# ziwang1121/IEEE

Hardware: NVIDIA B200
Metric: queries/sec (distmat+rank+CMC/mAP) (higher is better)
Workload: dtype f16x3 split of f32 (fp32-equivalent products, f32 accumulate); rank: u32/i32; AP: f64

## Files before the change

ieee_b200/csrc/rank.cu:

```cuda
#include "common.cuh"

namespace ieee {

static constexpr uint64_t kPadKey = ~uint64_t(0);

__device__ __forceinline__ void block_bitonic_sort(uint64_t* s, int n) {
  for (int k = 2; k <= n; k <<= 1) {
    for (int j = k >> 1; j > 0; j >>= 1) {
      __syncthreads();
      for (int i = threadIdx.x; i < n; i += blockDim.x) {
        const int p = i ^ j;
        if (p > i) {
          const uint64_t a = s[i], b = s[p];
          const bool up = (i & k) == 0;
          if ((a > b) == up) { s[i] = b; s[p] = a; }
        }
      }
    }
  }
  __syncthreads();
}
__host__ __device__ __forceinline__ int next_pow2(int x) {
  int p = 1;
  while (p < x) p <<= 1;
// ... 265 lines not shown
  int head = (int)(((16 - (addr & 15)) & 15) >> 2);
  if (head > G) head = G;
  const int nvec = (G - head) >> 2;
  const float4* rv = reinterpret_cast<const float4*>(row + head);
  if constexpr (MODE == COUNT_SEARCH_ATOMIC) {
    int g = tid;
    for (; g + 3 * NT < G; g += 4 * NT) {
      const float d0 = row[g], d1 = row[g + NT], d2 = row[g + 2 * NT], d3 = row[g + 3 * NT];
      count_visit_search<NT>(c, d0, (uint32_t)g);
      count_visit_search<NT>(c, d1, (uint32_t)(g + NT));
      count_visit_search<NT>(c, d2, (uint32_t)(g + 2 * NT));
      count_visit_search<NT>(c, d3, (uint32_t)(g + 3 * NT));
    }
    for (; g < G; g += NT) count_visit_search<NT>(c, row[g], (uint32_t)g);
    return;
  } else {
    auto one = [&](float d, uint32_t g) { if (count_visit<MODE, NT>(c, d)) count_fix<MODE, NT>(c, d, g); };
    for (int g = tid; g < head; g += NT) one(row[g], (uint32_t)g);
    int i = tid;
    for (; i + 3 * NT < nvec; i += 4 * NT) {
      const float4 a0 = __ldcs(rv + i), a1 = __ldcs(rv + i + NT), a2 = __ldcs(rv + i + 2 * NT), a3 = __ldcs(rv + i + 3 * NT);
      uint32_t g0 = (uint32_t)(head + 4 * i);
      one(a0.x, g0); one(a0.y, g0 + 1); one(a0.z, g0 + 2); one(a0.w, g0 + 3);
      g0 += 4 * NT;
      one(a1.x, g0); one(a1.y, g0 + 1); one(a1.z, g0 + 2); one(a1.w, g0 + 3);
      g0 += 4 * NT;
      one(a2.x, g0); one(a2.y, g0 + 1); one(a2.z, g0 + 2); one(a2.w, g0 + 3);
      g0 += 4 * NT;
      one(a3.x, g0); one(a3.y, g0 + 1); one(a3.z, g0 + 2); one(a3.w, g0 + 3);
    }
    for (; i < nvec; i += NT) {
      const float4 a = __ldcs(rv + i);
      const uint32_t g0 = (uint32_t)(head + 4 * i);
      one(a.x, g0); one(a.y, g0 + 1); one(a.z, g0 + 2); one(a.w, g0 + 3);
    }
    for (int g = head + 4 * nvec + tid; g < G; g += NT) one(row[g], (uint32_t)g);
  }
}

struct WarpCount {
  const uint64_t* T;
  const uint16_t* cell;
  uint8_t* col;
  const float* row;
  float lo, scale, top;
  uint32_t g_offset;
  int ties;
};

__host__ __device__ __forceinline__ uint16_t warp_cell_word(int first_bin, int n) {
  return (uint16_t)((first_bin << 7) | (n ? (((n - 1) << 1) | 1) : 0));
}

__device__ __forceinline__ uint32_t warp_cell_index(float d, float lo, float scale, float top) {
  return __float2uint_rd(fminf(fmaf(d - lo, scale, 1.0f), top));
}

__device__ __forceinline__ void warp_bump(WarpCount& c, uint32_t row_off, int delta) {
  atomicAdd(reinterpret_cast<int32_t*>(c.col + row_off), delta);
}

__device__ __forceinline__ void warp_fix(WarpCount& c, float d, uint32_t g) {
  const uint32_t ce = c.cell[warp_cell_index(d, c.lo, c.scale, c.top)];
  if (!(ce & 1u)) return;
  const int tent = (int)(ce >> 7), n = (int)((ce >> 1) & 63u) + 1;
  const uint64_t pe = pack_key(d, g + c.g_offset);
  const uint32_t ke = (uint32_t)(pe >> 32);
  int b = tent, same = 0;
  bool is_thr = false;
#pragma unroll 1
  for (int j = tent; j < tent + n; ++j) {
    const uint64_t t = c.T[j];
    b += (t < pe);
    same += ((uint32_t)(t >> 32) == ke);
    is_thr |= (t == pe);
  }
  if (!is_thr) c.ties += same;
  if (b != tent) {
    warp_bump(c, (uint32_t)tent << 7, -1);
    warp_bump(c, (uint32_t)b << 7, 1);
  }
}

__device__ __forceinline__ void warp_visit8(WarpCount& c, const float4& u, const float4& v, uint32_t& mask) {
  const float d[8] = {u.x, u.y, u.z, u.w, v.x, v.y, v.z, v.w};
  uint32_t ce[8];
#pragma unroll
  for (int e = 0; e < 8; ++e) ce[e] = c.cell[warp_cell_index(d[e], c.lo, c.scale, c.top)];
#pragma unroll
  for (int e = 0; e < 8; ++e) {
    warp_bump(c, ce[e] & 0xFF80u, 1);
    mask = mask * 2u + (ce[e] & 1u);
  }
}

__device__ __forceinline__ void warp_count_stream(WarpCount& c, int G, int lane, int wq, int team) {
  const float* __restrict__ row = c.row;
  const uintptr_t addr = reinterpret_cast<uintptr_t>(row);
  int head = (int)(((16 - (addr & 15)) & 15) >> 2);
  if (head > G) head = G;
  const int nvec = (G - head) >> 2;
  const float4* rv = reinterpret_cast<const float4*>(row + head);
  const int S = 32 * team, t0 = wq * 32 + lane;
  auto one = [&](int g) {
    const float d = row[g];
    const uint32_t ce = c.cell[warp_cell_index(d, c.lo, c.scale, c.top)];
    warp_bump(c, ce & 0xFF80u, 1);
    if (ce & 1u) warp_fix(c, d, (uint32_t)g);
  };
  for (int g = t0; g < head; g += S) one(g);
  int i = t0;
  bool have = i + 3 * S < nvec;
  float4 a0, a1, a2, a3;
  if (have) { a0 = __ldg(rv + i); a1 = __ldg(rv + i + S); a2 = __ldg(rv + i + 2 * S); a3 = __ldg(rv + i + 3 * S); }
  while (have) {
    const int in = i + 4 * S;
    const bool more = in + 3 * S < nvec;
    float4 n0 = a0, n1 = a1, n2 = a2, n3 = a3;
    if (more) { n0 = __ldg(rv + in); n1 = __ldg(rv + in + S); n2 = __ldg(rv + in + 2 * S); n3 = __ldg(rv + in + 3 * S); }
    uint32_t mask = 0;
    warp_visit8(c, a0, a1, mask);
    warp_visit8(c, a2, a3, mask);
#pragma unroll 1
    while (mask) {
      const int bit = 31 - __clz(mask);
      mask &= ~(1u << bit);
      const int e = 15 - bit;
      const int g = head + 4 * (i + (e >> 2) * S) + (e & 3);
      warp_fix(c, __ldg(row + g), (uint32_t)g);
    }
    a0 = n0; a1 = n1; a2 = n2; a3 = n3;
    i = in;
    have = more;
  }
  for (; i < nvec; i += S) {
    const int g0 = head + 4 * i;
    one(g0); one(g0 + 1); one(g0 + 2); one(g0 + 3);
  }
  for (int g = head + 4 * nvec + t0; g < G; g += S) one(g);
}

struct CountRow {
  int32_t* local;
  const PeerView* pv;
  int64_t slot_row;
  __device__ __forceinline__ void put(int idx, int32_t v) const {
    if (pv->shards == 0) { local[idx] = v; return; }
    for (int p = 0; p < pv->shards; ++p) reinterpret_cast<int32_t*>(pv->base[p] + pv->off_cnt)[slot_row + idx] = v;
  }
};
__device__ __forceinline__ CountRow count_row(int32_t* counts, int64_t q, int stride, const PeerView& pv) {
  CountRow r;
  r.local = counts ? counts + q * stride : nullptr;
  r.pv = &pv;
  r.slot_row = ((int64_t)pv.my * pv.Qb + q) * stride;
  return r;
}

constexpr int kWarpQ = 8;
constexpr int kCountTeamDefault = 1;
constexpr int kWarpRmax = 128;
struct WarpMisc { float lo, scale, top; int R, use_lut, ties; uint32_t kmax; int pad; };
__host__ __device__ inline int warp_smem_per_query(int rmax, int wpq) {
  return ((rmax * 8 + (rmax + 2) * 4 + (kLutCells + 4) * 2 + 32 + wpq * (rmax + 2) * 32 * 4) + 15) & ~15;
}

template <int WPQ>
__global__ void __launch_bounds__(32 * kWarpQ)
rank_count_warp_kernel(const float* __restrict__ distmat, int64_t ld, int64_t Q, int G, int64_t g_offset, int shards, int cap,
                       int out_cap, int rmax, const uint64_t* __restrict__ rel_all, const int32_t* __restrict__ n_rel,
                       const uint64_t* __restrict__ junk, const int32_t* __restrict__ n_junk, int32_t* __restrict__ counts,
                       unsigned long long* __restrict__ ties_out, const PeerView pv) {
  static_assert(WPQ == 1 || WPQ == 2 || WPQ == 4 || WPQ == kWarpQ, "1, 2, 4 or all 8 warps of the CTA per query");
  if (pv.shards) peer_signal_and_wait(pv, 0);
  constexpr bool kTeam = WPQ > 1;
  constexpr int kTeams = kWarpQ / WPQ;
  extern __shared__ __align__(16) uint8_t ws_raw[];
  const int lane = threadIdx.x & 31, w = threadIdx.x >> 5;
  const int team = w / WPQ, wq = w % WPQ;
  uint8_t* mine = ws_raw + size_t(team) * warp_smem_per_query(rmax, WPQ);
  uint64_t* T = reinterpret_cast<uint64_t*>(mine);
  int32_t* hist = reinterpret_cast<int32_t*>(mine + rmax * 8);
  uint16_t* cell = reinterpret_cast<uint16_t*>(hist + rmax + 2);
  WarpMisc* misc = reinterpret_cast<WarpMisc*>(cell + kLutCells + 4);
  int32_t* priv = reinterpret_cast<int32_t*>(misc + 1) + size_t(wq) * (rmax + 2) * 32;
  auto team_sync = [&]() {
    if constexpr (WPQ == kWarpQ) __syncthreads();
    else if constexpr (kTeam) asm volatile("bar.sync %0, %1;" ::"r"(team + 1), "r"(32 * WPQ) : "memory");
    else __syncwarp();
  };
  const int64_t q = (int64_t)blockIdx.x * kTeams + team;
  if (q >= Q) return;
  const int stride = out_cap + 2;
  const CountRow out = count_row(counts, q, stride, pv);
  const int nj = n_junk[q];
  int Rtot = 0, my_n = 0, my_base = 0;
  const bool lanes_cover_shards = shards <= 32;
  if (lanes_cover_shards) {
    if (lane < shards) my_n = (int)rel_all[((int64_t)lane * Q + q) * (cap + 1) + cap];
    int incl = my_n;
#pragma unroll
    for (int o = 1; o < 32; o <<= 1) { const int v = __shfl_up_sync(0xffffffffu, incl, o); if (lane >= o) incl += v; }
    my_base = incl - my_n;
    Rtot = __shfl_sync(0xffffffffu, incl, 31);
  } else {
    for (int s = 0; s < shards; ++s) Rtot += (int)rel_all[((int64_t)s * Q + q) * (cap + 1) + cap];
  }
  if (lane == 0 && wq == 0) {
    out.put(stride - 1, nj); out.put(stride - 2, n_rel[q]);
    if (ties_out != nullptr && (unsigned long long)Rtot > ties_out[1]) atomicMax(ties_out + 1, (unsigned long long)Rtot);
  }
  if (Rtot == 0 || Rtot > rmax) return;
  const int R = Rtot;
  const int L = lut_cells_for(G);
  if (wq == 0) {
    uint64_t* Tin = reinterpret_cast<uint64_t*>(priv);
    if (lanes_cover_shards) {
      for (int idx0 = 0; idx0 < R; idx0 += 32) {
        const int idx = idx0 + lane;
        int s_mine = -1, i_mine = 0;
        for (int s = 0; s < shards; ++s) {
          const int b = __shfl_sync(0xffffffffu, my_base, s), n = __shfl_sync(0xffffffffu, my_n, s);
          if (idx >= b && idx < b + n) { s_mine = s; i_mine = idx - b; }
        }
        if (s_mine >= 0) Tin[idx] = rel_all[((int64_t)s_mine * Q + q) * (cap + 1) + i_mine];
      }
    } else {
      int base = 0;
      for (int s = 0; s < shards; ++s) {
        const uint64_t* src = rel_all + ((int64_t)s * Q + q) * (cap + 1);
        const int n = (int)src[cap];
        for (int i = lane; i < n; i += 32) Tin[base + i] = src[i];
        base += n;
      }
    }
    __syncwarp();
    for (int k = lane; k < R; k += 32) {
      const uint64_t me = Tin[k];
      int pos = 0;
      for (int j = 0; j < R; ++j) pos += (Tin[j] < me);
      T[pos] = me;
    }
    __syncwarp();
    const uint32_t kmin = (uint32_t)(T[0] >> 32), kmax = (uint32_t)(T[R - 1] >> 32);
    const float lo = key_to_float(kmin), hi = key_to_float(kmax);
    const float span = hi - lo;
    bool use_lut = (kmax != 0xFFFFFFFFu) && isfinite(lo) && isfinite(hi);
    const float scale = use_lut ? fminf(((float)L - 0.5f) / span, 1.2676506e30f ) : 0.f;
    const float top = (float)(L + 1);
    if (use_lut) {
      uint16_t* tcell = reinterpret_cast<uint16_t*>(hist);
      for (int k = lane; k < R; k += 32) {
        const uint32_t ci = warp_cell_index(key_to_float((uint32_t)(T[k] >> 32)), lo, scale, top);
        tcell[k] = (uint16_t)min(max(ci, 1u), (uint32_t)L);
      }
      __syncwarp();
      uint32_t* cell32 = reinterpret_cast<uint32_t*>(cell);
      for (int i = lane; i < (L + 4) / 2; i += 32) cell32[i] = 0;
      __syncwarp();
      bool crowded = false;
      for (int k = lane; k < R; k += 32) {
        const int cidx = tcell[k];
        if (k == 0 || (int)tcell[k - 1] != cidx) {
          int n = 1;
          while (k + n < R && (int)tcell[k + n] == cidx) ++n;
          crowded |= n > 64;
          cell[cidx] = warp_cell_word(k, min(n, 64));
        }
      }
      __syncwarp();
      const int chunk = (L + 2 + 31) / 32;
      const int c0 = lane * chunk, c1 = min(c0 + chunk, L + 2);
      int last = -1;
      for (int i = c0; i < c1; ++i) {
        const uint32_t cw = cell[i];
        if (cw & 1u) last = (int)(cw >> 7) + (int)((cw >> 1) & 63u) + 1;
      }
      const uint32_t have = __ballot_sync(0xffffffffu, last >= 0) & ((1u << lane) - 1u);
      const int src = have ? 31 - __clz(have) : lane;
      const int below = __shfl_sync(0xffffffffu, last, src);
      int run = have ? below : 0;
      for (int i = c0; i < c1; ++i) {
        const uint32_t cw = cell[i];
        if (cw & 1u) run = (int)(cw >> 7) + (int)((cw >> 1) & 63u) + 1;
        else cell[i] = (i == L + 1) ? warp_cell_word(R + 1, 0) : warp_cell_word(run, 0);
      }
      if (__any_sync(0xffffffffu, crowded)) use_lut = false;
      __syncwarp();
    }
    for (int i = lane; i < R + 2; i += 32) hist[i] = 0;
    if (lane == 0) {
      misc->lo = lo; misc->scale = scale; misc->top = top; misc->R = R; misc->use_lut = use_lut ? 1 : 0;
      misc->ties = 0; misc->kmax = kmax;
    }
    __syncwarp();
  }
  for (int i = lane; i < (R + 2) * 32; i += 32) priv[i] = 0;
  team_sync();
  const float lo = misc->lo, scale = misc->scale, top = misc->top;
  const bool use_lut = misc->use_lut != 0;
  const uint32_t kmax = misc->kmax;
  const float* row = distmat + q * ld;
  int tie_local = 0;
  if (use_lut) {
    WarpCount c;
    c.T = T; c.cell = cell; c.col = reinterpret_cast<uint8_t*>(priv + lane); c.row = row;
    c.lo = lo; c.scale = scale; c.top = top; c.g_offset = (uint32_t)g_offset; c.ties = 0;
    warp_count_stream(c, G, lane, wq, WPQ);
    tie_local = c.ties;
  } else {
    CountCtx c;
    c.T = T; c.cell = nullptr; c.hist = hist; c.priv = priv + lane;
    c.lo = lo; c.hi = 0.f; c.scale = scale; c.kmax = kmax; c.R = R; c.trash = R + 1; c.L = L;
    c.g_offset = (uint32_t)g_offset; c.ties = 0;
    count_stream<COUNT_SEARCH_ATOMIC, 32 * WPQ>(c, row, G, wq * 32 + lane);
    tie_local = c.ties;
  }
  __syncwarp();
  if (use_lut) {
    for (int b = lane; b <= R; b += 32) {
      int sum = 0;
      for (int j = 0; j < 32; ++j) sum += priv[b * 32 + ((j + lane) & 31)];
      if constexpr (kTeam) atomicAdd(&hist[b], sum); else hist[b] = sum;
    }
  }
  if constexpr (kTeam) {
    for (int o = 16; o > 0; o >>= 1) tie_local += __shfl_xor_sync(0xffffffffu, tie_local, o);
    if (lane == 0 && tie_local != 0) atomicAdd(&misc->ties, tie_local);
    tie_local = 0;
  }
  team_sync();
  if (wq != 0) return;
  for (int i = lane; i < nj; i += 32) {
    const uint64_t pe = junk[q * cap + i];
    const uint32_t ke = (uint32_t)(pe >> 32);
    if (ke > kmax) continue;
    int a = 0, e = R;
    while (a < e) { const int m = (a + e) >> 1; if (T[m] < pe) a = m + 1; else e = m; }
    for (int j = a; j < R && (uint32_t)(T[j] >> 32) == ke; ++j) tie_local--;
    for (int j = a - 1; j >= 0 && (uint32_t)(T[j] >> 32) == ke; --j) tie_local--;
    atomicSub(&hist[a], 1);
  }
  for (int o = 16; o > 0; o >>= 1) tie_local += __shfl_xor_sync(0xffffffffu, tie_local, o);
  if constexpr (kTeam) tie_local += misc->ties;
  __syncwarp();
  int carry = 0;
  for (int base = 0; base < R; base += 32) {
    const int k = base + lane;
    const int v = k < R ? hist[k] : 0;
    int incl = v;
#pragma unroll
    for (int o = 1; o < 32; o <<= 1) { int n = __shfl_up_sync(0xffffffffu, incl, o); if (lane >= o) incl += n; }
    if (k < R) {
      const int64_t gi = (int64_t)(uint32_t)T[k] - g_offset;
      out.put(k, carry + incl - ((gi >= 0 && gi < G) ? 1 : 0));
    }
    carry += __shfl_sync(0xffffffffu, incl, 31);
  }
  if (lane == 0 && ties_out != nullptr && tie_local != 0) atomicAdd(ties_out, (unsigned long long)(long long)tie_local);
}

__global__ void __launch_bounds__(kCountThreads, 6)
rank_count_kernel(const float* __restrict__ distmat, int64_t ld, int64_t Q, int G, int64_t g_offset, int shards, int cap,
                  int out_cap, int Rp, const uint64_t* __restrict__ rel_all, const int32_t* __restrict__ n_rel,
                  const uint64_t* __restrict__ junk, const int32_t* __restrict__ n_junk, int32_t* __restrict__ counts,
                  unsigned long long* __restrict__ ties_out, const PeerView pv) {
  extern __shared__ __align__(16) uint8_t cs_raw[];
  if (pv.shards) peer_signal_and_wait(pv, 0);
  const CountSmemPlan plan = count_smem_plan(Rp);
  uint64_t* T = reinterpret_cast<uint64_t*>(cs_raw);
  int32_t* hist = reinterpret_cast<int32_t*>(cs_raw + plan.hist_off);
  uint32_t* cell = reinterpret_cast<uint32_t*>(cs_raw + plan.cell_off);
  int32_t* misc = reinterpret_cast<int32_t*>(cs_raw + plan.misc_off);
  int32_t* priv = reinterpret_cast<int32_t*>(cs_raw + plan.priv_off);
  const int64_t q = blockIdx.x;
  const int tid = threadIdx.x;
  const int stride = out_cap + 2;
  const CountRow out = count_row(counts, q, stride, pv);
  int Rtot = 0;
  for (int s = 0; s < shards; ++s) Rtot += (int)rel_all[((int64_t)s * Q + q) * (cap + 1) + cap];
  if (tid == 0 && ties_out != nullptr && (unsigned long long)Rtot > ties_out[1]) atomicMax(ties_out + 1, (unsigned long long)Rtot);
  if (Rtot > out_cap) {
    if (tid == 0) { out.put(stride - 1, n_junk[q]); out.put(stride - 2, n_rel[q]); }
    return;
  }

  if (tid == 0) { misc[0] = 0; misc[1] = 0; }
  for (int i = tid; i < kLutCells + 2; i += kCountThreads) cell[i] = 0;
  __syncthreads();
  const bool stage_in_priv = size_t(Rp) * 8 <= size_t(plan.priv_bins) * kCountThreads * 4;
  uint64_t* Tin = stage_in_priv ? reinterpret_cast<uint64_t*>(priv) : T;
  for (int s = 0; s < shards; ++s) {
    const uint64_t* src = rel_all + ((int64_t)s * Q + q) * (cap + 1);
    const int n = (int)src[cap];
    __shared__ int base_s;
    if (tid == 0) { base_s = misc[0]; misc[0] += n; }
    __syncthreads();
    for (int i = tid; i < n; i += kCountThreads) Tin[base_s + i] = src[i];
    __syncthreads();
  }
  const int R = misc[0];
  const int nj = n_junk[q];
  if (tid == 0) { out.put(stride - 1, nj); out.put(stride - 2, n_rel[q]); }
  if (R == 0) return;
  if (stage_in_priv && R <= 512) {
    for (int k = tid; k < R; k += kCountThreads) {
      const uint64_t me = Tin[k];
      int pos = 0;
      for (int j = 0; j < R; ++j) pos += (Tin[j] < me);
      T[pos] = me;
    }
  } else {
// ... 94 lines not shown
    if (lane == 31) wsum[w] = incl;
    __syncthreads();
    int woff = carry;
    for (int i = 0; i < w; ++i) woff += wsum[i];
    if (k < R) {
      const int64_t gi = (int64_t)(uint32_t)T[k] - g_offset;
      out.put(k, woff + incl - ((gi >= 0 && gi < G) ? 1 : 0));
    }
    __syncthreads();
    if (tid == kCountThreads - 1) carry = woff + incl;
    __syncthreads();
  }
  if (tid == 0 && ties_out != nullptr && misc[1] != 0) atomicAdd(ties_out, (unsigned long long)(long long)misc[1]);
}

static int count_warp_max_g() {
  static int v = -1;
  if (v < 0) {
    const char* e = getenv("IEEE_B200_COUNT_WARP_MAX_G");
    v = e ? atoi(e) : 65536;
    if (v < 0) v = 65536;
  }
  return v;
}

static int g_count_team = -1;
static int count_team_mid() {
  if (g_count_team < 0) {
    const char* e = getenv("IEEE_B200_COUNT_WPQ");
    const int v = e ? atoi(e) : kCountTeamDefault;
    g_count_team = (v == 1 || v == 2 || v == 4 || v == 8) ? v : kCountTeamDefault;
  }
  return g_count_team;
}
int set_count_team(int wpq) {
  const int prev = count_team_mid();
  if (wpq == 1 || wpq == 2 || wpq == 4 || wpq == 8) g_count_team = wpq;
  return prev;
}

size_t rank_count_smem(int shards, int cap) { return count_smem_plan(next_pow2(max(shards * cap, 2))).total; }

int rank_count(const float* distmat, int64_t ld, int64_t Q, int64_t G, int64_t g_offset, int shards, int cap, int out_cap,
               const uint64_t* rel_all, const int32_t* n_rel, const uint64_t* junk, const int32_t* n_junk,
               int32_t* counts, unsigned long long* ties, cudaStream_t stream, const PeerView* peers) {
  const PeerView pv = peers ? *peers : no_peers();
  IEEE_REQUIRE(distmat && rel_all && n_rel && junk && n_junk && (counts || pv.shards), "rank_count: null pointer");
  IEEE_REQUIRE(Q >= 0 && G > 0 && G < (int64_t(1) << 31) && ld >= G && shards >= 1 && cap >= 1 && out_cap >= 0,
               "rank_count: bad shape");
  if (Q == 0) return IEEE_OK;
  if (out_cap == 0 || out_cap > shards * cap) out_cap = shards * cap;
  if (out_cap <= kWarpRmax && !(g_debug_flags & 16)) {
    const int rmax = (out_cap + 1) & ~1;
    const int wpq = G > count_warp_max_g() ? kWarpQ : (G >= 4096 ? count_team_mid() : 1);
    const int teams = kWarpQ / wpq;
    const size_t wsmem = size_t(teams) * warp_smem_per_query(rmax, wpq);
    const unsigned grid = (unsigned)((Q + teams - 1) / teams);
#define IEEE_COUNT_LAUNCH(W)                                                                                                   \
  do {                                                                                                                         \
    IEEE_ENSURE_DYN_SMEM(rank_count_warp_kernel<W>, wsmem);                                                                    \
    rank_count_warp_kernel<W><<<grid, 32 * kWarpQ, wsmem, stream>>>(distmat, ld, Q, (int)G, g_offset, shards, cap, out_cap, rmax, \
                                                                    rel_all, n_rel, junk, n_junk, counts, ties, pv);           \
  } while (0)
    if (wpq == kWarpQ) IEEE_COUNT_LAUNCH(kWarpQ);
    else if (wpq == 4) IEEE_COUNT_LAUNCH(4);
    else if (wpq == 2) IEEE_COUNT_LAUNCH(2);
    else IEEE_COUNT_LAUNCH(1);
#undef IEEE_COUNT_LAUNCH
    count_launch(1, "rank_count_warp_kernel");
    IEEE_CUDA_CHECK(cudaGetLastError());
    return IEEE_OK;
  }
  const int Rp = next_pow2(max(out_cap, 2));
  const size_t smem = count_smem_plan(Rp).total;
  IEEE_REQUIRE(smem <= 200 * 1024, "rank_count: %d relevant items per query exceed the shared-memory budget", out_cap);
  IEEE_ENSURE_DYN_SMEM(rank_count_kernel, smem);
  rank_count_kernel<<<(unsigned)Q, kCountThreads, smem, stream>>>(distmat, ld, Q, (int)G, g_offset, shards, cap, out_cap, Rp, rel_all,
                                                                  n_rel, junk, n_junk, counts, ties, pv);
  count_launch(1, "rank_count_kernel");
  IEEE_CUDA_CHECK(cudaGetLastError());
  return IEEE_OK;
}

int rank_gather(const float* distmat, int64_t ld, int64_t Q, int64_t G, const int64_t* q_pids, const int64_t* q_camids,
                const int64_t* g_camids, const void* group, int64_t g_offset, int32_t cap, uint64_t* rel, int32_t* n_rel,
                uint64_t* junk, int32_t* n_junk, int32_t* overflow, cudaStream_t stream, const PeerView* peers) {
  const PeerView pv = peers ? *peers : no_peers();
  IEEE_REQUIRE(distmat && q_pids && q_camids && g_camids && group && (rel || pv.shards) && n_rel && junk && n_junk && overflow,
               "rank_gather: null pointer");
  IEEE_REQUIRE(Q >= 0 && G > 0 && ld >= G && cap >= 1, "rank_gather: bad shape");
  IEEE_REQUIRE(g_offset >= 0 && g_offset + G <= (int64_t(1) << 32), "rank_gather: global gallery index must fit 32 bits");
  if (Q == 0) return IEEE_OK;
  GroupView v = group_view(group, G);
  const int stage = (pv.shards != 0 && cap <= 255) ? 1 : 0;
  const size_t smem = stage ? size_t(8) * (cap + 1) * 8 : 0;
  rank_gather_kernel<<<(unsigned)((Q + 7) / 8), 256, smem, stream>>>(distmat, ld, Q, G, q_pids, q_camids, g_camids, v.keys, v.cnt,
                                                                     v.off, v.members, v.T, g_offset, cap, rel, n_rel, junk, n_junk,
                                                                     overflow, pv, stage);
  count_launch(1, "rank_gather_kernel");
  IEEE_CUDA_CHECK(cudaGetLastError());
  return IEEE_OK;
}

__device__ __forceinline__ void query_metrics(const int32_t* __restrict__ counts, int64_t q, int64_t G_total, int stride,
                                              int max_rank, double* ap, int32_t* first, int32_t* is_short, double* inp) {
  const int32_t* c = counts + q * stride;
  const int R = c[stride - 2];
  if (R == 0) {
    ap[q] = 0.0; first[q] = -1; is_short[q] = 0;
    if (inp) inp[q] = 0.0;
    return;
  }
  if (inp) inp[q] = (double)R / ((double)c[R - 1] + 1.0);
  double s = 0.0;
  for (int k = 0; k < R; ++k) s += (double)(k + 1) / ((double)c[k] + 1.0);
  ap[q] = s / (double)R;
  first[q] = c[0];
  const int64_t kept = G_total - (int64_t)c[stride - 1];
  is_short[q] = kept < max_rank ? 1 : 0;
}

__global__ void __launch_bounds__(256) rank_query_kernel(const int32_t* __restrict__ counts,
// ... 588 lines not shown
```

Measured before the change: 4.336 million.

## Count ranks with one CTA per query and packed 16-bit private histograms

```diff
diff --git a/ieee_b200/csrc/rank.cu b/ieee_b200/csrc/rank.cu
--- a/ieee_b200/csrc/rank.cu
+++ b/ieee_b200/csrc/rank.cu
@@ -341,14 +341,25 @@
   return (uint16_t)((first_bin << 7) | (n ? (((n - 1) << 1) | 1) : 0));
 }
 
+__host__ __device__ __forceinline__ int count_rows(int bins, bool packed) { return packed ? (bins + 1) / 2 : bins; }
+
+__host__ __device__ inline bool count16_fits(int64_t G, int nw) {
+  return 4 * ((G + 128 * nw - 1) / (128 * nw)) + 2 < 65536;
+}
+
 __device__ __forceinline__ uint32_t warp_cell_index(float d, float lo, float scale, float top) {
   return __float2uint_rd(fminf(fmaf(d - lo, scale, 1.0f), top));
 }
 
-__device__ __forceinline__ void warp_bump(WarpCount& c, uint32_t row_off, int delta) {
-  atomicAdd(reinterpret_cast<int32_t*>(c.col + row_off), delta);
-}
-
+template <bool kPacked>
+__device__ __forceinline__ void warp_bump(WarpCount& c, uint32_t bin7, int delta) {
+  if constexpr (kPacked)
+    atomicAdd(reinterpret_cast<uint32_t*>(c.col + ((bin7 >> 1) & ~127u)), (uint32_t)delta << ((bin7 >> 3) & 16u));
+  else
+    atomicAdd(reinterpret_cast<int32_t*>(c.col + bin7), delta);
+}
+
+template <bool kPacked>
 __device__ __forceinline__ void warp_fix(WarpCount& c, float d, uint32_t g) {
   const uint32_t ce = c.cell[warp_cell_index(d, c.lo, c.scale, c.top)];
   if (!(ce & 1u)) return;
@@ -366,11 +377,12 @@
   }
   if (!is_thr) c.ties += same;
   if (b != tent) {
-    warp_bump(c, (uint32_t)tent << 7, -1);
-    warp_bump(c, (uint32_t)b << 7, 1);
-  }
-}
-
+    warp_bump<kPacked>(c, (uint32_t)tent << 7, -1);
+    warp_bump<kPacked>(c, (uint32_t)b << 7, 1);
+  }
+}
+
+template <bool kPacked>
 __device__ __forceinline__ void warp_visit8(WarpCount& c, const float4& u, const float4& v, uint32_t& mask) {
   const float d[8] = {u.x, u.y, u.z, u.w, v.x, v.y, v.z, v.w};
   uint32_t ce[8];
@@ -378,11 +390,12 @@
   for (int e = 0; e < 8; ++e) ce[e] = c.cell[warp_cell_index(d[e], c.lo, c.scale, c.top)];
 #pragma unroll
   for (int e = 0; e < 8; ++e) {
-    warp_bump(c, ce[e] & 0xFF80u, 1);
+    warp_bump<kPacked>(c, ce[e] & 0xFF80u, 1);
     mask = mask * 2u + (ce[e] & 1u);
   }
 }
 
+template <bool kPacked, bool kPipe = true>
 __device__ __forceinline__ void warp_count_stream(WarpCount& c, int G, int lane, int wq, int team) {
   const float* __restrict__ row = c.row;
   const uintptr_t addr = reinterpret_cast<uintptr_t>(row);
@@ -394,8 +407,8 @@
   auto one = [&](int g) {
     const float d = row[g];
     const uint32_t ce = c.cell[warp_cell_index(d, c.lo, c.scale, c.top)];
-    warp_bump(c, ce & 0xFF80u, 1);
-    if (ce & 1u) warp_fix(c, d, (uint32_t)g);
+    warp_bump<kPacked>(c, ce & 0xFF80u, 1);
+    if (ce & 1u) warp_fix<kPacked>(c, d, (uint32_t)g);
   };
   for (int g = t0; g < head; g += S) one(g);
   int i = t0;
@@ -406,18 +419,19 @@
     const int in = i + 4 * S;
     const bool more = in + 3 * S < nvec;
     float4 n0 = a0, n1 = a1, n2 = a2, n3 = a3;
-    if (more) { n0 = __ldg(rv + in); n1 = __ldg(rv + in + S); n2 = __ldg(rv + in + 2 * S); n3 = __ldg(rv + in + 3 * S); }
+    if (kPipe && more) { n0 = __ldg(rv + in); n1 = __ldg(rv + in + S); n2 = __ldg(rv + in + 2 * S); n3 = __ldg(rv + in + 3 * S); }
     uint32_t mask = 0;
-    warp_visit8(c, a0, a1, mask);
-    warp_visit8(c, a2, a3, mask);
+    warp_visit8<kPacked>(c, a0, a1, mask);
+    warp_visit8<kPacked>(c, a2, a3, mask);
 #pragma unroll 1
     while (mask) {
       const int bit = 31 - __clz(mask);
       mask &= ~(1u << bit);
       const int e = 15 - bit;
       const int g = head + 4 * (i + (e >> 2) * S) + (e & 3);
-      warp_fix(c, __ldg(row + g), (uint32_t)g);
-    }
+      warp_fix<kPacked>(c, __ldg(row + g), (uint32_t)g);
+    }
+    if (!kPipe && more) { n0 = __ldg(rv + in); n1 = __ldg(rv + in + S); n2 = __ldg(rv + in + 2 * S); n3 = __ldg(rv + in + 3 * S); }
     a0 = n0; a1 = n1; a2 = n2; a3 = n3;
     i = in;
     have = more;
@@ -447,206 +461,305 @@
 }
 
 constexpr int kWarpQ = 8;
-constexpr int kCountTeamDefault = 1;
+constexpr int kCountTeamDefault = 8;
 constexpr int kWarpRmax = 128;
-struct WarpMisc { float lo, scale, top; int R, use_lut, ties; uint32_t kmax; int pad; };
-__host__ __device__ inline int warp_smem_per_query(int rmax, int wpq) {
-  return ((rmax * 8 + (rmax + 2) * 4 + (kLutCells + 4) * 2 + 32 + wpq * (rmax + 2) * 32 * 4) + 15) & ~15;
-}
-
-template <int WPQ>
+
+struct CountSmem {
+  uint64_t* T;
+  int32_t* hist;
+  uint16_t* cell;
+  int32_t* misc;
+  int32_t* priv;
+};
+__host__ __device__ inline int count_query_smem(int rmax, int nw, bool packed) {
+  return ((rmax * 8 + (rmax + 2) * 4 + (kLutCells + 4) * 2 + 64 + nw * count_rows(rmax + 2, packed) * 128) + 15) & ~15;
+}
+__device__ __forceinline__ CountSmem count_smem(uint8_t* base, int rmax) {
+  CountSmem s;
+  s.T = reinterpret_cast<uint64_t*>(base);
+  s.hist = reinterpret_cast<int32_t*>(base + rmax * 8);
+  s.cell = reinterpret_cast<uint16_t*>(s.hist + rmax + 2);
+  s.misc = reinterpret_cast<int32_t*>(s.cell + kLutCells + 4);
+  s.priv = s.misc + 16;
+  return s;
+}
+
+struct ShardLists { int R, my_n, my_base; };
+__device__ __forceinline__ ShardLists shard_lists(const uint64_t* __restrict__ rel_all, int64_t Q, int64_t q, int cap, int shards,
+                                                  int lane) {
+  ShardLists s{0, 0, 0};
+  if (shards <= 32) {
+    if (lane < shards) s.my_n = (int)rel_all[((int64_t)lane * Q + q) * (cap + 1) + cap];
+    int incl = s.my_n;
+#pragma unroll
+    for (int o = 1; o < 32; o <<= 1) { const int v = __shfl_up_sync(0xffffffffu, incl, o); if (lane >= o) incl += v; }
+    s.my_base = incl - s.my_n;
+    s.R = __shfl_sync(0xffffffffu, incl, 31);
+  } else {
+    for (int sh = 0; sh < shards; ++sh) s.R += (int)rel_all[((int64_t)sh * Q + q) * (cap + 1) + cap];
+  }
+  return s;
+}
+
+template <bool kCta>
+__device__ __forceinline__ void count_sync() {
+  if constexpr (kCta) __syncthreads(); else __syncwarp();
+}
+
+struct CountSetup { float lo, scale, top; uint32_t kmax; bool use_lut; };
+
+template <bool kCta>
+__device__ __forceinline__ CountSetup count_setup(const CountSmem& s, const uint64_t* __restrict__ rel_all, int64_t Q, int64_t q,
+                                                  int cap, int shards, const ShardLists& sl, int L, int t, int nt) {
+  const int lane = t & 31, R = sl.R;
+  uint64_t* Tin = reinterpret_cast<uint64_t*>(s.priv);
+  if (shards <= 32) {
+    for (int idx0 = t - lane; idx0 < R; idx0 += nt) {
+      const int idx = idx0 + lane;
+      int s_mine = -1, i_mine = 0;
+      for (int sh = 0; sh < shards; ++sh) {
+        const int b = __shfl_sync(0xffffffffu, sl.my_base, sh), n = __shfl_sync(0xffffffffu, sl.my_n, sh);
+        if (idx >= b && idx < b + n) { s_mine = sh; i_mine = idx - b; }
+      }
+      if (s_mine >= 0) Tin[idx] = rel_all[((int64_t)s_mine * Q + q) * (cap + 1) + i_mine];
+    }
+  } else {
+    int base = 0;
+    for (int sh = 0; sh < shards; ++sh) {
+      const uint64_t* src = rel_all + ((int64_t)sh * Q + q) * (cap + 1);
+      const int n = (int)src[cap];
+      for (int i = t; i < n; i += nt) Tin[base + i] = src[i];
+      base += n;
+    }
+  }
+  count_sync<kCta>();
+  for (int k = t; k < R; k += nt) {
+    const uint64_t me = Tin[k];
+    int pos = 0;
+    for (int j = 0; j < R; ++j) pos += (Tin[j] < me);
+    s.T[pos] = me;
+  }
+  count_sync<kCta>();
+  CountSetup st;
+  const uint32_t kmin = (uint32_t)(s.T[0] >> 32);
+  st.kmax = (uint32_t)(s.T[R - 1] >> 32);
+  st.lo = key_to_float(kmin);
+  const float hi = key_to_float(st.kmax);
+  const float span = hi - st.lo;
+  st.use_lut = (st.kmax != 0xFFFFFFFFu) && isfinite(st.lo) && isfinite(hi);
+  st.scale = st.use_lut ? fminf(((float)L - 0.5f) / span, 1.2676506e30f ) : 0.f;
+  st.top = (float)(L + 1);
+  if (st.use_lut) {
+    uint16_t* tcell = reinterpret_cast<uint16_t*>(s.hist);
+    uint16_t* cell = s.cell;
+    for (int k = t; k < R; k += nt) {
+      const uint32_t ci = warp_cell_index(key_to_float((uint32_t)(s.T[k] >> 32)), st.lo, st.scale, st.top);
+      tcell[k] = (uint16_t)min(max(ci, 1u), (uint32_t)L);
+    }
+    uint32_t* cell32 = reinterpret_cast<uint32_t*>(cell);
+    for (int i = t; i < (L + 4) / 2; i += nt) cell32[i] = 0;
+    count_sync<kCta>();
+    bool crowded = false;
+    for (int k = t; k < R; k += nt) {
+      const int cidx = tcell[k];
+      if (k == 0 || (int)tcell[k - 1] != cidx) {
+        int n = 1;
+        while (k + n < R && (int)tcell[k + n] == cidx) ++n;
+        crowded |= n > 64;
+        cell[cidx] = warp_cell_word(k, min(n, 64));
+      }
+    }
+    count_sync<kCta>();
+    const int chunk = (L + 2 + nt - 1) / nt;
+    const int c0 = min(t * chunk, L + 2), c1 = min(c0 + chunk, L + 2);
+    int last = -1;
+    for (int i = c0; i < c1; ++i) {
+      const uint32_t cw = cell[i];
+      if (cw & 1u) last = (int)(cw >> 7) + (int)((cw >> 1) & 63u) + 1;
+    }
+    int incl = last;
+#pragma unroll
+    for (int o = 1; o < 32; o <<= 1) { const int v = __shfl_up_sync(0xffffffffu, incl, o); if (lane >= o) incl = max(incl, v); }
+    int below = __shfl_up_sync(0xffffffffu, incl, 1);
+    if (lane == 0) below = -1;
+    if constexpr (kCta) {
+      if (lane == 31) s.misc[t >> 5] = incl;
+      __syncthreads();
+      for (int i = 0; i < (t >> 5); ++i) below = max(below, s.misc[i]);
+    }
+    int run = max(below, 0);
+    for (int i = c0; i < c1; ++i) {
+      const uint32_t cw = cell[i];
+      if (cw & 1u) run = (int)(cw >> 7) + (int)((cw >> 1) & 63u) + 1;
+      else cell[i] = (i == L + 1) ? warp_cell_word(R + 1, 0) : warp_cell_word(run, 0);
+    }
+    if constexpr (kCta) {
+      crowded = __syncthreads_or(crowded) != 0;
+    } else {
+      crowded = __any_sync(0xffffffffu, crowded);
+      __syncwarp();
+    }
+    if (crowded) st.use_lut = false;
+  }
+  for (int i = t; i < R + 2; i += nt) s.hist[i] = 0;
+  return st;
+}
+
+__device__ __forceinline__ int count_remove_junk(const CountSmem& s, const uint64_t* __restrict__ junk_q, int nj, int R, uint32_t kmax,
+                                                 int t, int nt) {
+  int ties = 0;
+  for (int i = t; i < nj; i += nt) {
+    const uint64_t pe = junk_q[i];
+    const uint32_t ke = (uint32_t)(pe >> 32);
+    if (ke > kmax) continue;
+    int a = 0, e = R;
+    while (a < e) { const int m = (a + e) >> 1; if (s.T[m] < pe) a = m + 1; else e = m; }
+    for (int j = a; j < R && (uint32_t)(s.T[j] >> 32) == ke; ++j) ties--;
+    for (int j = a - 1; j >= 0 && (uint32_t)(s.T[j] >> 32) == ke; --j) ties--;
+    atomicSub(&s.hist[a], 1);
+  }
+  return ties;
+}
+
+__device__ __forceinline__ void count_write_row(const CountSmem& s, const CountRow& out, int R, int64_t g_offset, int G, int lane) {
+  int carry = 0;
+  for (int base = 0; base < R; base += 32) {
+    const int k = base + lane;
+    const int v = k < R ? s.hist[k] : 0;
+    int incl = v;
+#pragma unroll
+    for (int o = 1; o < 32; o <<= 1) { int n = __shfl_up_sync(0xffffffffu, incl, o); if (lane >= o) incl += n; }
+    if (k < R) {
+      const int64_t gi = (int64_t)(uint32_t)s.T[k] - g_offset;
+      out.put(k, carry + incl - ((gi >= 0 && gi < G) ? 1 : 0));
+    }
+    carry += __shfl_sync(0xffffffffu, incl, 31);
+  }
+}
+
+template <bool kPacked, typename Add>
+__device__ __forceinline__ void warp_fold(const int32_t* priv, int R, int lane, Add add) {
+  for (int r = lane; r < count_rows(R + 1, kPacked); r += 32) {
+    int s0 = 0, s1 = 0;
+    for (int j = 0; j < 32; ++j) {
+      const uint32_t v = (uint32_t)priv[r * 32 + ((j + lane) & 31)];
+      if constexpr (kPacked) { s0 += (int)(v & 0xFFFFu); s1 += (int)(v >> 16); } else s0 += (int)v;
+    }
+    if constexpr (kPacked) {
+      add(2 * r, s0);
+      if (2 * r + 1 <= R) add(2 * r + 1, s1);
+    } else {
+      add(r, s0);
+    }
+  }
+}
+
 __global__ void __launch_bounds__(32 * kWarpQ)
 rank_count_warp_kernel(const float* __restrict__ distmat, int64_t ld, int64_t Q, int G, int64_t g_offset, int shards, int cap,
                        int out_cap, int rmax, const uint64_t* __restrict__ rel_all, const int32_t* __restrict__ n_rel,
                        const uint64_t* __restrict__ junk, const int32_t* __restrict__ n_junk, int32_t* __restrict__ counts,
                        unsigned long long* __restrict__ ties_out, const PeerView pv) {
-  static_assert(WPQ == 1 || WPQ == 2 || WPQ == 4 || WPQ == kWarpQ, "1, 2, 4 or all 8 warps of the CTA per query");
   if (pv.shards) peer_signal_and_wait(pv, 0);
-  constexpr bool kTeam = WPQ > 1;
-  constexpr int kTeams = kWarpQ / WPQ;
   extern __shared__ __align__(16) uint8_t ws_raw[];
   const int lane = threadIdx.x & 31, w = threadIdx.x >> 5;
-  const int team = w / WPQ, wq = w % WPQ;
-  uint8_t* mine = ws_raw + size_t(team) * warp_smem_per_query(rmax, WPQ);
-  uint64_t* T = reinterpret_cast<uint64_t*>(mine);
-  int32_t* hist = reinterpret_cast<int32_t*>(mine + rmax * 8);
-  uint16_t* cell = reinterpret_cast<uint16_t*>(hist + rmax + 2);
-  WarpMisc* misc = reinterpret_cast<WarpMisc*>(cell + kLutCells + 4);
-  int32_t* priv = reinterpret_cast<int32_t*>(misc + 1) + size_t(wq) * (rmax + 2) * 32;
-  auto team_sync = [&]() {
-    if constexpr (WPQ == kWarpQ) __syncthreads();
-    else if constexpr (kTeam) asm volatile("bar.sync %0, %1;" ::"r"(team + 1), "r"(32 * WPQ) : "memory");
-    else __syncwarp();
-  };
-  const int64_t q = (int64_t)blockIdx.x * kTeams + team;
+  const int64_t q = (int64_t)blockIdx.x * kWarpQ + w;
   if (q >= Q) return;
+  const CountSmem s = count_smem(ws_raw + size_t(w) * count_query_smem(rmax, 1, false), rmax);
   const int stride = out_cap + 2;
   const CountRow out = count_row(counts, q, stride, pv);
   const int nj = n_junk[q];
-  int Rtot = 0, my_n = 0, my_base = 0;
-  const bool lanes_cover_shards = shards <= 32;
-  if (lanes_cover_shards) {
-    if (lane < shards) my_n = (int)rel_all[((int64_t)lane * Q + q) * (cap + 1) + cap];
-    int incl = my_n;
-#pragma unroll
-    for (int o = 1; o < 32; o <<= 1) { const int v = __shfl_up_sync(0xffffffffu, incl, o); if (lane >= o) incl += v; }
-    my_base = incl - my_n;
-    Rtot = __shfl_sync(0xffffffffu, incl, 31);
-  } else {
-    for (int s = 0; s < shards; ++s) Rtot += (int)rel_all[((int64_t)s * Q + q) * (cap + 1) + cap];
-  }
-  if (lane == 0 && wq == 0) {
+  const ShardLists sl = shard_lists(rel_all, Q, q, cap, shards, lane);
+  if (lane == 0) {
     out.put(stride - 1, nj); out.put(stride - 2, n_rel[q]);
-    if (ties_out != nullptr && (unsigned long long)Rtot > ties_out[1]) atomicMax(ties_out + 1, (unsigned long long)Rtot);
-  }
-  if (Rtot == 0 || Rtot > rmax) return;
-  const int R = Rtot;
+    if (ties_out != nullptr && (unsigned long long)sl.R > ties_out[1]) atomicMax(ties_out + 1, (unsigned long long)sl.R);
+  }
+  const int R = sl.R;
+  if (R == 0 || R > rmax) return;
   const int L = lut_cells_for(G);
-  if (wq == 0) {
-    uint64_t* Tin = reinterpret_cast<uint64_t*>(priv);
-    if (lanes_cover_shards) {
-      for (int idx0 = 0; idx0 < R; idx0 += 32) {
-        const int idx = idx0 + lane;
-        int s_mine = -1, i_mine = 0;
-        for (int s = 0; s < shards; ++s) {
-          const int b = __shfl_sync(0xffffffffu, my_base, s), n = __shfl_sync(0xffffffffu, my_n, s);
-          if (idx >= b && idx < b + n) { s_mine = s; i_mine = idx - b; }
-        }
-        if (s_mine >= 0) Tin[idx] = rel_all[((int64_t)s_mine * Q + q) * (cap + 1) + i_mine];
-      }
-    } else {
-      int base = 0;
-      for (int s = 0; s < shards; ++s) {
-        const uint64_t* src = rel_all + ((int64_t)s * Q + q) * (cap + 1);
-        const int n = (int)src[cap];
-        for (int i = lane; i < n; i += 32) Tin[base + i] = src[i];
-        base += n;
-      }
-    }
-    __syncwarp();
-    for (int k = lane; k < R; k += 32) {
-      const uint64_t me = Tin[k];
-      int pos = 0;
-      for (int j = 0; j < R; ++j) pos += (Tin[j] < me);
-      T[pos] = me;
-    }
-    __syncwarp();
-    const uint32_t kmin = (uint32_t)(T[0] >> 32), kmax = (uint32_t)(T[R - 1] >> 32);
-    const float lo = key_to_float(kmin), hi = key_to_float(kmax);
-    const float span = hi - lo;
-    bool use_lut = (kmax != 0xFFFFFFFFu) && isfinite(lo) && isfinite(hi);
-    const float scale = use_lut ? fminf(((float)L - 0.5f) / span, 1.2676506e30f ) : 0.f;
-    const float top = (float)(L + 1);
-    if (use_lut) {
-      uint16_t* tcell = reinterpret_cast<uint16_t*>(hist);
-      for (int k = lane; k < R; k += 32) {
-        const uint32_t ci = warp_cell_index(key_to_float((uint32_t)(T[k] >> 32)), lo, scale, top);
-        tcell[k] = (uint16_t)min(max(ci, 1u), (uint32_t)L);
-      }
-      __syncwarp();
-      uint32_t* cell32 = reinterpret_cast<uint32_t*>(cell);
-      for (int i = lane; i < (L + 4) / 2; i += 32) cell32[i] = 0;
-      __syncwarp();
-      bool crowded = false;
-      for (int k = lane; k < R; k += 32) {
-        const int cidx = tcell[k];
-        if (k == 0 || (int)tcell[k - 1] != cidx) {
-          int n = 1;
-          while (k + n < R && (int)tcell[k + n] == cidx) ++n;
-          crowded |= n > 64;
-          cell[cidx] = warp_cell_word(k, min(n, 64));
-        }
-      }
-      __syncwarp();
-      const int chunk = (L + 2 + 31) / 32;
-      const int c0 = lane * chunk, c1 = min(c0 + chunk, L + 2);
-      int last = -1;
-      for (int i = c0; i < c1; ++i) {
-        const uint32_t cw = cell[i];
-        if (cw & 1u) last = (int)(cw >> 7) + (int)((cw >> 1) & 63u) + 1;
-      }
-      const uint32_t have = __ballot_sync(0xffffffffu, last >= 0) & ((1u << lane) - 1u);
-      const int src = have ? 31 - __clz(have) : lane;
-      const int below = __shfl_sync(0xffffffffu, last, src);
-      int run = have ? below : 0;
-      for (int i = c0; i < c1; ++i) {
-        const uint32_t cw = cell[i];
-        if (cw & 1u) run = (int)(cw >> 7) + (int)((cw >> 1) & 63u) + 1;
-        else cell[i] = (i == L + 1) ? warp_cell_word(R + 1, 0) : warp_cell_word(run, 0);
-      }
-      if (__any_sync(0xffffffffu, crowded)) use_lut = false;
-      __syncwarp();
-    }
-    for (int i = lane; i < R + 2; i += 32) hist[i] = 0;
-    if (lane == 0) {
-      misc->lo = lo; misc->scale = scale; misc->top = top; misc->R = R; misc->use_lut = use_lut ? 1 : 0;
-      misc->ties = 0; misc->kmax = kmax;
-    }
-    __syncwarp();
-  }
-  for (int i = lane; i < (R + 2) * 32; i += 32) priv[i] = 0;
-  team_sync();
-  const float lo = misc->lo, scale = misc->scale, top = misc->top;
-  const bool use_lut = misc->use_lut != 0;
-  const uint32_t kmax = misc->kmax;
+  const CountSetup st = count_setup<false>(s, rel_all, Q, q, cap, shards, sl, L, lane, 32);
+  for (int i = lane; i < (R + 2) * 32; i += 32) s.priv[i] = 0;
+  __syncwarp();
   const float* row = distmat + q * ld;
   int tie_local = 0;
-  if (use_lut) {
+  if (st.use_lut) {
     WarpCount c;
-    c.T = T; c.cell = cell; c.col = reinterpret_cast<uint8_t*>(priv + lane); c.row = row;
-    c.lo = lo; c.scale = scale; c.top = top; c.g_offset = (uint32_t)g_offset; c.ties = 0;
-    warp_count_stream(c, G, lane, wq, WPQ);
+    c.T = s.T; c.cell = s.cell; c.col = reinterpret_cast<uint8_t*>(s.priv + lane); c.row = row;
+    c.lo = st.lo; c.scale = st.scale; c.top = st.top; c.g_offset = (uint32_t)g_offset; c.ties = 0;
+    warp_count_stream<false>(c, G, lane, 0, 1);
     tie_local = c.ties;
   } else {
     CountCtx c;
-    c.T = T; c.cell = nullptr; c.hist = hist; c.priv = priv + lane;
-    c.lo = lo; c.hi = 0.f; c.scale = scale; c.kmax = kmax; c.R = R; c.trash = R + 1; c.L = L;
+    c.T = s.T; c.cell = nullptr; c.hist = s.hist; c.priv = nullptr;
+    c.lo = st.lo; c.hi = 0.f; c.scale = st.scale; c.kmax = st.kmax; c.R = R; c.trash = R + 1; c.L = L;
     c.g_offset = (uint32_t)g_offset; c.ties = 0;
-    count_stream<COUNT_SEARCH_ATOMIC, 32 * WPQ>(c, row, G, wq * 32 + lane);
+    count_stream<COUNT_SEARCH_ATOMIC, 32>(c, row, G, lane);
     tie_local = c.ties;
   }
   __syncwarp();
-  if (use_lut) {
-    for (int b = lane; b <= R; b += 32) {
-      int sum = 0;
-      for (int j = 0; j < 32; ++j) sum += priv[b * 32 + ((j + lane) & 31)];
-      if constexpr (kTeam) atomicAdd(&hist[b], sum); else hist[b] = sum;
-    }
-  }
-  if constexpr (kTeam) {
-    for (int o = 16; o > 0; o >>= 1) tie_local += __shfl_xor_sync(0xffffffffu, tie_local, o);
-    if (lane == 0 && tie_local != 0) atomicAdd(&misc->ties, tie_local);
-    tie_local = 0;
-  }
-  team_sync();
-  if (wq != 0) return;
-  for (int i = lane; i < nj; i += 32) {
-    const uint64_t pe = junk[q * cap + i];
-    const uint32_t ke = (uint32_t)(pe >> 32);
-    if (ke > kmax) continue;
-    int a = 0, e = R;
-    while (a < e) { const int m = (a + e) >> 1; if (T[m] < pe) a = m + 1; else e = m; }
-    for (int j = a; j < R && (uint32_t)(T[j] >> 32) == ke; ++j) tie_local--;
-    for (int j = a - 1; j >= 0 && (uint32_t)(T[j] >> 32) == ke; --j) tie_local--;
-    atomicSub(&hist[a], 1);
-  }
+  if (st.use_lut) warp_fold<false>(s.priv, R, lane, [&](int b, int v) { s.hist[b] = v; });
+  __syncwarp();
+  tie_local += count_remove_junk(s, junk + q * cap, nj, R, st.kmax, lane, 32);
   for (int o = 16; o > 0; o >>= 1) tie_local += __shfl_xor_sync(0xffffffffu, tie_local, o);
-  if constexpr (kTeam) tie_local += misc->ties;
   __syncwarp();
-  int carry = 0;
-  for (int base = 0; base < R; base += 32) {
-    const int k = base + lane;
-    const int v = k < R ? hist[k] : 0;
-    int incl = v;
-#pragma unroll
-    for (int o = 1; o < 32; o <<= 1) { int n = __shfl_up_sync(0xffffffffu, incl, o); if (lane >= o) incl += n; }
-    if (k < R) {
-      const int64_t gi = (int64_t)(uint32_t)T[k] - g_offset;
-      out.put(k, carry + incl - ((gi >= 0 && gi < G) ? 1 : 0));
-    }
-    carry += __shfl_sync(0xffffffffu, incl, 31);
-  }
+  count_write_row(s, out, R, g_offset, G, lane);
   if (lane == 0 && ties_out != nullptr && tie_local != 0) atomicAdd(ties_out, (unsigned long long)(long long)tie_local);
+}
+
+template <int NW, bool kPacked, bool kPipe = true, int MB = (kPacked ? 6 : 5)>
+__global__ void __launch_bounds__(32 * kWarpQ, MB)
+rank_count_cta_kernel(const float* __restrict__ distmat, int64_t ld, int64_t Q, int G, int64_t g_offset, int shards, int cap,
+                      int out_cap, int rmax, const uint64_t* __restrict__ rel_all, const int32_t* __restrict__ n_rel,
+                      const uint64_t* __restrict__ junk, const int32_t* __restrict__ n_junk, int32_t* __restrict__ counts,
+                      unsigned long long* __restrict__ ties_out, const PeerView pv) {
+  static_assert(NW == 2 || NW == 4 || NW == kWarpQ, "2, 4 or 8 warps per query");
+  constexpr int NT = 32 * NW;
+  if (pv.shards) peer_signal_and_wait(pv, 0);
+  extern __shared__ __align__(16) uint8_t ws_raw[];
+  const int tid = threadIdx.x, lane = tid & 31, w = tid >> 5;
+  const int64_t q = blockIdx.x;
+  const CountSmem s = count_smem(ws_raw, rmax);
+  const int stride = out_cap + 2;
+  const CountRow out = count_row(counts, q, stride, pv);
+  const int nj = n_junk[q];
+  const ShardLists sl = shard_lists(rel_all, Q, q, cap, shards, lane);
+  if (tid == 0) {
+    out.put(stride - 1, nj); out.put(stride - 2, n_rel[q]);
+    if (ties_out != nullptr && (unsigned long long)sl.R > ties_out[1]) atomicMax(ties_out + 1, (unsigned long long)sl.R);
+  }
+  const int R = sl.R;
+  if (R == 0 || R > rmax) return;
+  const int L = lut_cells_for(G);
+  const CountSetup st = count_setup<true>(s, rel_all, Q, q, cap, shards, sl, L, tid, NT);
+  const int rows = count_rows(R + 2, kPacked);
+  for (int i = tid; i < NW * rows * 32; i += NT) s.priv[i] = 0;
+  if (tid == 0) s.misc[8] = 0;
+  __syncthreads();
+  int32_t* priv = s.priv + w * rows * 32;
+  const float* row = distmat + q * ld;
+  int tie_local = 0;
+  if (st.use_lut) {
+    WarpCount c;
+    c.T = s.T; c.cell = s.cell; c.col = reinterpret_cast<uint8_t*>(priv + lane); c.row = row;
+    c.lo = st.lo; c.scale = st.scale; c.top = st.top; c.g_offset = (uint32_t)g_offset; c.ties = 0;
+    warp_count_stream<kPacked, kPipe>(c, G, lane, w, NW);
+    tie_local = c.ties;
+  } else {
+    CountCtx c;
+    c.T = s.T; c.cell = nullptr; c.hist = s.hist; c.priv = nullptr;
+    c.lo = st.lo; c.hi = 0.f; c.scale = st.scale; c.kmax = st.kmax; c.R = R; c.trash = R + 1; c.L = L;
+    c.g_offset = (uint32_t)g_offset; c.ties = 0;
+    count_stream<COUNT_SEARCH_ATOMIC, NT>(c, row, G, tid);
+    tie_local = c.ties;
+  }
+  __syncwarp();
+  if (st.use_lut) warp_fold<kPacked>(priv, R, lane, [&](int b, int v) { if (v != 0) atomicAdd(&s.hist[b], v); });
+  tie_local += count_remove_junk(s, junk + q * cap, nj, R, st.kmax, tid, NT);
+  for (int o = 16; o > 0; o >>= 1) tie_local += __shfl_xor_sync(0xffffffffu, tie_local, o);
+  if (lane == 0 && tie_local != 0) atomicAdd(&s.misc[8], tie_local);
+  __syncthreads();
+  if (w != 0) return;
+  count_write_row(s, out, R, g_offset, G, lane);
+  if (lane == 0 && ties_out != nullptr && s.misc[8] != 0) atomicAdd(ties_out, (unsigned long long)(long long)s.misc[8]);
 }
 
 __global__ void __launch_bounds__(kCountThreads, 6)
@@ -847,22 +960,37 @@
   if (out_cap == 0 || out_cap > shards * cap) out_cap = shards * cap;
   if (out_cap <= kWarpRmax && !(g_debug_flags & 16)) {
     const int rmax = (out_cap + 1) & ~1;
-    const int wpq = G > count_warp_max_g() ? kWarpQ : (G >= 4096 ? count_team_mid() : 1);
-    const int teams = kWarpQ / wpq;
-    const size_t wsmem = size_t(teams) * warp_smem_per_query(rmax, wpq);
-    const unsigned grid = (unsigned)((Q + teams - 1) / teams);
-#define IEEE_COUNT_LAUNCH(W)                                                                                                   \
+    const bool long_row = G > count_warp_max_g();
+    int nw = long_row ? kWarpQ : (G >= 4096 ? count_team_mid() : 1);
+    bool packed = !long_row && nw > 1;
+    if (getenv("IEEE_B200_TMP_COUNT_VARIANT") && atoi(getenv("IEEE_B200_TMP_COUNT_VARIANT")) == 3) packed = false;
+    if (packed && !count16_fits(G, nw)) { nw = kWarpQ; packed = false; }
+    if (nw == 1) {
+      const size_t smem = size_t(kWarpQ) * count_query_smem(rmax, 1, false);
+      IEEE_ENSURE_DYN_SMEM(rank_count_warp_kernel, smem);
+      rank_count_warp_kernel<<<(unsigned)((Q + kWarpQ - 1) / kWarpQ), 32 * kWarpQ, smem, stream>>>(
+          distmat, ld, Q, (int)G, g_offset, shards, cap, out_cap, rmax, rel_all, n_rel, junk, n_junk, counts, ties, pv);
+      count_launch(1, "rank_count_warp_kernel");
+    } else {
+      const size_t smem = count_query_smem(rmax, nw, packed);
+#define IEEE_COUNT_CTA(W, ...)                                                                                                   \
   do {                                                                                                                         \
-    IEEE_ENSURE_DYN_SMEM(rank_count_warp_kernel<W>, wsmem);                                                                    \
-    rank_count_warp_kernel<W><<<grid, 32 * kWarpQ, wsmem, stream>>>(distmat, ld, Q, (int)G, g_offset, shards, cap, out_cap, rmax, \
-                                                                    rel_all, n_rel, junk, n_junk, counts, ties, pv);           \
+    IEEE_ENSURE_DYN_SMEM((rank_count_cta_kernel<W, __VA_ARGS__>), smem);                                                                 \
+    rank_count_cta_kernel<W, __VA_ARGS__><<<(unsigned)Q, 32 * W, smem, stream>>>(distmat, ld, Q, (int)G, g_offset, shards, cap, out_cap,  \
+                                                                       rmax, rel_all, n_rel, junk, n_junk, counts, ties, pv);  \
   } while (0)
-    if (wpq == kWarpQ) IEEE_COUNT_LAUNCH(kWarpQ);
-    else if (wpq == 4) IEEE_COUNT_LAUNCH(4);
-    else if (wpq == 2) IEEE_COUNT_LAUNCH(2);
-    else IEEE_COUNT_LAUNCH(1);
-#undef IEEE_COUNT_LAUNCH
-    count_launch(1, "rank_count_warp_kernel");
+      static const int tmpv = getenv("IEEE_B200_TMP_COUNT_VARIANT") ? atoi(getenv("IEEE_B200_TMP_COUNT_VARIANT")) : 0;
+      if (!packed && nw == kWarpQ) IEEE_COUNT_CTA(kWarpQ, false);
+      else if (nw == kWarpQ && tmpv == 1) IEEE_COUNT_CTA(kWarpQ, true, true, 5);
+      else if (nw == kWarpQ && tmpv == 2) IEEE_COUNT_CTA(kWarpQ, true, false, 6);
+      else if (nw == kWarpQ && tmpv == 4) IEEE_COUNT_CTA(kWarpQ, true, false, 8);
+      else if (nw == kWarpQ && tmpv == 5) IEEE_COUNT_CTA(kWarpQ, true, false, 5);
+      else if (nw == 4) IEEE_COUNT_CTA(4, true);
+      else if (nw == 2) IEEE_COUNT_CTA(2, true);
+      else IEEE_COUNT_CTA(kWarpQ, true);
+#undef IEEE_COUNT_CTA
+      count_launch(1, "rank_count_cta_kernel");
+    }
     IEEE_CUDA_CHECK(cudaGetLastError());
     return IEEE_OK;
   }
diff --git a/profiles/count_stage_probe.py b/profiles/count_stage_probe.py
--- /dev/null
+++ b/profiles/count_stage_probe.py
@@ -0,0 +1,113 @@
+import argparse
+import hashlib
+import os
+import subprocess
+import sys
+
+import numpy as np
+import torch
+
+sys.path.insert(0, os.path.dirname(os.path.dirname(os.path.abspath(__file__))))
+from ieee_b200 import _lib
+from ieee_b200.engine import PackedFeatures, feature_center, packed_distmat, shard_bounds
+from ieee_b200.metrics.rank import GalleryLabels, RankStages
+from ieee_b200.testing import make_retrieval_set, market1501_shaped
+
+ap = argparse.ArgumentParser()
+ap.add_argument("--reps", type=int, default=30)
+ap.add_argument("--shapes", default="market,n8,c4")
+ap.add_argument("--team", type=int, default=0, help="ieee_set_count_team before timing (0: leave the default)")
+args = ap.parse_args()
+dev = torch.device("cuda")
+lib = _lib.load()
+if args.team:
+    lib.ieee_set_count_team(args.team)
+try:
+    card = subprocess.run(["nvidia-smi", "--query-gpu=name,power.limit", "--format=csv,noheader", "-i", "0"],
+                          capture_output=True, text=True, timeout=60).stdout.strip()
+except Exception as e:
+    card = "%s (nvidia-smi: %s)" % (torch.cuda.get_device_name(0), e)
+print("card: %s; library: %s; team %d" % (card, _lib.LIB_PATH, lib.ieee_set_count_team(-1)), flush=True)
+
+
+def dist(qf, gf, center=True):
+    c = feature_center(qf) if center else None
+    q, g = PackedFeatures(qf, "euclidean", False, "f16x3", c), PackedFeatures(gf, "euclidean", False, "f16x3", c)
+    out = torch.empty((qf.shape[0], (gf.shape[0] + 31) // 32 * 32), device=dev)[:, :gf.shape[0]]
+    packed_distmat(q, g, out)
+    return out
+
+
+def market():
+    s = market1501_shaped(seed=1)
+    d = dist(s.qf.to(dev), s.gf.to(dev))
+    qp, qc = torch.from_numpy(s.q_pids).to(dev), torch.from_numpy(s.q_camids).to(dev)
+    gal = GalleryLabels(torch.from_numpy(s.g_pids).to(dev), torch.from_numpy(s.g_camids).to(dev), dev)
+    st = RankStages(d.shape[0], gal.list_cap(qp), 1, dev)
+    st.gather(d, qp, qc, gal)
+    return st, d, 0, None
+
+
+def n8():
+    N = 8
+    s = market1501_shaped(num_q=3368 * N)
+    Q, G = s.qf.shape[0], s.gf.shape[0]
+    qf = s.qf.to(dev)
+    qp, qc = torch.from_numpy(s.q_pids).to(dev), torch.from_numpy(s.q_camids).to(dev)
+    bounds = [shard_bounds(G, N, r) for r in range(N)]
+    gals = [GalleryLabels(torch.from_numpy(s.g_pids[g0:g1].copy()).to(dev), torch.from_numpy(s.g_camids[g0:g1].copy()).to(dev), dev)
+            for g0, g1 in bounds]
+    cap = max(gal.list_cap(qp) for gal in gals)
+    rels, d0 = [], None
+    for (g0, g1), gal in zip(bounds, gals):
+        d = dist(qf, s.gf[g0:g1].to(dev), center=False)
+        st = RankStages(Q, cap, N, dev)
+        st.gather(d, qp, qc, gal, g0)
+        rels.append(st.rel)
+        d0 = d if d0 is None else d0
+    rel_all = torch.stack(rels).contiguous()
+    probe = RankStages(Q, cap, N, dev)
+    probe.gather(d0, qp, qc, gals[0], 0)
+    probe.count(d0, gals[0].G, 0, rel_all)
+    st = RankStages(Q, cap, N, dev, int(probe.flags[2].item()))
+    st.gather(d0, qp, qc, gals[0], 0)
+    return st, d0, 0, rel_all
+
+
+def c4():
+    Q, G = 8192, 125000
+    s = make_retrieval_set(Q, G, 12500, 8, dim=256, sigma=2.0, seed=3)
+    d = dist(s.qf.to(dev), s.gf.to(dev), center=False)
+    qp, qc = torch.from_numpy(s.q_pids).to(dev), torch.from_numpy(s.q_camids).to(dev)
+    gal = GalleryLabels(torch.from_numpy(s.g_pids).to(dev), torch.from_numpy(s.g_camids).to(dev), dev)
+    st = RankStages(Q, gal.list_cap(qp), 1, dev)
+    st.gather(d, qp, qc, gal)
+    return st, d, 0, None
+
+
+flush = torch.empty(256 << 20, dtype=torch.uint8, device=dev)
+for name in args.shapes.split(","):
+    st, d, g0, rel_all = {"market": market, "n8": n8, "c4": c4}[name]()
+    Q, G = d.shape
+    for _ in range(3):
+        st.flags.zero_()
+        st.count(d, G, g0, rel_all)
+    ts = []
+    a, b = torch.cuda.Event(enable_timing=True), torch.cuda.Event(enable_timing=True)
+    for _ in range(args.reps):
+        flush.zero_()
+        a.record()
+        st.count(d, G, g0, rel_all)
+        b.record()
+        torch.cuda.synchronize()
+        ts.append(a.elapsed_time(b) * 1e3)
+    st.flags.zero_()
+    st.count(d, G, g0, rel_all)
+    torch.cuda.synchronize()
+    digest = hashlib.sha1(st.counts.cpu().numpy().tobytes() + st.flags[1:3].cpu().numpy().tobytes()).hexdigest()[:16]
+    med, mn = float(np.median(ts)), min(ts)
+    print("%-6s Q %6d x G %6d  width %3d: median %8.1f us  min %8.1f us  (%5.0f / %5.0f GB/s)  ties %d  longest %d  digest %s"
+          % (name, Q, G, st.width, med, mn, 4.0 * Q * G / med / 1e3, 4.0 * Q * G / mn / 1e3, int(st.flags[1]), int(st.flags[2]),
+             digest), flush=True)
+    del st, d, rel_all
+    torch.cuda.empty_cache()
```

New measurement: 4.214 million, median of 6. 2.8% lower.
